# AdrianoEttari/DiffusionRemoteSensing

Hardware: AMD Instinct MI355X
Metric: unet_denoise_steps_per_s (higher is better)
Workload: dtype f16 main + block-scaled fp6 (e2m3) cross terms of tap pairs on the wide 3x3 layers (FL, 11 of 11 launches of the dominant kernel); split bf16 x3 (hi + lo) everywhere else; f32 accumulate

## Files before the change

diffusionremotesensing_amd/csrc/drs_common.h:

```cpp
#pragma once
#include <hip/hip_runtime.h>
#include <stdint.h>
#include <stddef.h>

#include "../../include/drs_hip.h"

#define DRS_MAX_TAPS 9
#define DRS_TAPMODE_CONVT 2

struct TapConv {
  const float* in;
  int in_cs, in_co;
  int N, H, W, Cin;
  const float* w;
  const void* w_aux;
  const float* bias;
  float* out;
  int out_cs, out_co;
  int OH, OW, Cout;
  int TH, TW;
  int in_stride, out_scale, out_oy, out_ox;
  int ntaps;
  int dy[DRS_MAX_TAPS], dx[DRS_MAX_TAPS], wtap[DRS_MAX_TAPS];
  int wtaps_total;
// ... 135 lines not shown
  const float* in; int in_cs, in_co;
  int N, LH, LW, Cc, Ch;
  const void* w;
  const float* bias;
  const float* res; int res_cs, res_co;
  const float* eh;
  const float* ev;
  float* out; int out_cs, out_co;
  float* out2; int out2_cs, out2_co;
  const float* post2; int post2_cs;
  const float* fuse_w; const float* fuse_b; float* fuse_out; int fuse_dim;
  int fuse_acc;
  int proj;
  const void* zero_line;
  unsigned* fault;
};
bool drs_upfuse_proj_supported(int Cc, int Ch, int fuse_dim);
size_t drs_upfuse_proj_weight_bytes(int Cc);
int drs_launch_upfuse_proj_pack(const float* vp, const float* t_w, int Cc, int Ch, int fuse_dim, void* dst, hipStream_t s);
int drs_launch_upfuse_proj(const UpFuseDesc& d, hipStream_t s);
int drs_launch_upfuse_fold_proj(const float* v_w, const float* v_b, const float* fw, const float* fb, int fuse_dim, int Cc, int Ch,
                                float* dst_w, float* dst_b, hipStream_t s);

struct ResBlock0Desc {
  const float* x;
  const void* w1; const float* b1;
  const float* temb; int temb_cs;
  const void* w2; const float* b2;
  const void* ws; const float* bs;
  float* out;
  int N, H, W;
  const void* zero_line;
  unsigned* fault;
};
bool drs_resblock0_supported(int Cin, int Cout, int H, int W);
int drs_launch_resblock0(const ResBlock0Desc& d, hipStream_t s);
struct UpFuseEdgeDesc {
  const float* in; int in_cs, in_co; int N, LH, LW, Cc, Ch;
  const float* rt; const float* rl; const float* bt;
  float* eh; float* ev;
  const void* wimg;
  const void* zero_line;
};
bool drs_upfuse_supported(int Cc, int Ch, int LH, int LW);
size_t drs_upfuse_weight_bytes(int Cc, int Ch);
size_t drs_upfuse_aux_floats(int Cc, int Ch);
size_t drs_upfuse_edge_image_bytes(int Cc, int Ch);
int drs_launch_upfuse_pack(const float* v_w, const float* v_b, const float* t_w, const float* t_b, int Cc, int Ch, void* dst_w,
                           float* dst_aux, void* dst_edge, hipStream_t s);
int drs_launch_upfuse_edges(const UpFuseEdgeDesc& d, hipStream_t s);
int drs_launch_upfuse(const UpFuseDesc& d, hipStream_t s);
int drs_launch_nchw_to_sp(const float* src, float* dst, int N, int C, int H, int W, hipStream_t s);

int drs_launch_sp_add_rowvec(const float* src, float* dst, const float* vec, int vec_stride, int N, long long pix_per_image,
                             int C, hipStream_t s);
bool drs_tapconv_sp8_supported(const TapConv& d, int impl);
bool drs_tapconv_sp_supported(const TapConv& d, int impl);
int drs_launch_conv3x3_direct_sp(const TapConv& d, hipStream_t s);
int drs_launch_fold_proj(const float* w, int cin_total, int cin_off, int Cmid, int Cin, const float* fw, int fuse_dim, float* dst,
// ... 64 lines not shown
```

diffusionremotesensing_amd/csrc/plan.hip:

```cpp
#include <stdarg.h>
#include <stdio.h>
#include <stdlib.h>
#include <string.h>
#include <cxxabi.h>
#include <algorithm>
#include <map>
#include <memory>
#include <mutex>
#include <string>
#include <utility>
#include <vector>

#include "drs_common.h"

static thread_local char g_err[512] = "";
void DrsErr::set(const char* fmt, ...) {
  va_list ap;
  va_start(ap, fmt);
  vsnprintf(g_err, sizeof(g_err), fmt, ap);
  va_end(ap);
}
extern "C" const char* drs_last_error(void) { return g_err; }
extern "C" int drs_abi_version(void) { return 7; }

// ... 377 lines not shown
  int t_PA = -1;
  size_t o_eh = 0, o_ev = 0;
};

}

struct drs_plan {
  drs_unet_config cfg;
  std::vector<Param> params;
  std::vector<ConvLayer*> convs;
  std::vector<PlanarConv*> planars;
  std::vector<Mlp*> mlps;
  std::vector<WsTensor> tensors;

  PlanarConv rrdb[7];
  PlanarConv stem0, stemc;
  ResBlock enc[4];
  ConvLayer downs[3];
  DecStage dec[3];
  ConvLayer output;

  size_t packed_bytes = 0, ws_bytes = 0;
  size_t o_inv_freq = 0, o_mlp_table = 0, o_out_w = 0, o_out_b = 0, o_label = 0, o_zero = 0, o_fault = 0;
  bool sp = false;
  int t_XT[3] = {-1, -1, -1};
  int label_emb = -1;
  int temb_total = 0;
  std::vector<long long> mlp_table_host;
  std::vector<const void*> param_ptrs;
  size_t o_bn_sums = 0, bn_sums_bytes = 0, o_red = 0, red_bytes = 0;
  bool fl = false;
  bool fl_disabled = false;
  int fl_slots = 0;
  size_t o_fl_flags = 0;
  bool packed_ok = false;
  const void* packed_ptr = nullptr;
  unsigned* fault_ptr = nullptr;

  struct OpRec { std::string name; double flops, bytes; hipEvent_t e0, e1; };
  bool profiling = false;
  std::vector<OpRec> ops;
  struct LaunchRec { std::string op, kernel; };
  std::vector<LaunchRec> launches;
  std::string cur_op;

  size_t o_lr[3], o_up, o_temb;
// ... 207 lines not shown
    }
  }
  if (p->fl) {
    for (ConvLayer* L : p->convs)
      if (L->fl_slot >= 0) { L->fl_img_off = cur; cur += align_up(drs_fl_image_bytes(L->Cout, L->Cin, L->taps)); }
    for (int i = 0; i < 2; ++i)
      if (p->dec[i].ah_fl_slot >= 0) { p->dec[i].ah_fl_img_off = cur; cur += align_up(drs_fl_image_bytes(kUp[i + 1], kUp[i + 1], 9)); }
    p->o_fl_flags = cur; cur += align_up((size_t)p->fl_slots * 8);
  }
  for (PlanarConv* L : p->planars) {
    L->w_off = cur; cur += align_up((size_t)L->Cout * L->Cin * 9 * 4);
    L->b_off = cur; cur += align_up((size_t)L->Cout * 4);
  }
  for (Mlp* m : p->mlps) {
    m->o_w1 = cur; cur += align_up((size_t)m->dim * 100 * 4);
    m->o_b1 = cur; cur += align_up((size_t)m->dim * 4);
    m->o_w2 = cur; cur += align_up((size_t)m->dim * m->dim * 4);
    m->o_b2 = cur; cur += align_up((size_t)m->dim * 4);
  }
  p->o_mlp_table = cur; cur += align_up(p->mlps.size() * 6 * sizeof(long long));
  p->o_label = cur; cur += align_up((size_t)(cfg.num_classes > 0 ? cfg.num_classes : 0) * 100 * 4);
  p->o_out_w = cur; cur += align_up((size_t)cfg.out_dim * kUp[3] * 4);
  p->o_out_b = cur; cur += align_up((size_t)cfg.out_dim * 4);
  p->o_zero = cur; cur += 256;
  p->o_fault = cur; cur += 256;
  p->packed_bytes = cur;
}

static void plan_eval_workspace(drs_plan* p, size_t& ws) {
  const drs_unet_config& cfg = p->cfg;
  const int B = cfg.batch, Bl = cfg.lr_batch, H = cfg.height, W = cfg.width, h = H / cfg.magnification, w = W / cfg.magnification;
  const int CCw = cfg.cond_channels > 0 ? cfg.cond_channels : 1;
  for (int i = 0; i < 3; ++i) { p->o_lr[i] = ws; ws += align_up((size_t)Bl * CCw * h * w * 4); }
  p->o_temb = ws; ws += align_up((size_t)B * p->temb_total * 4);
  p->t_lrenc = p->T(cond_encoder_name(cfg), ws, Bl, CCw, h, w, true);
  p->t_up = p->T("upsampled_lr_img", ws, Bl, CCw, H, W, true);
  p->t_cond = p->T("cond", ws, Bl, kDown[0], H, W);
  p->t_x0 = p->T("x0", ws, B, kDown[0], H, W);
  for (int i = 0; i < 4; ++i) {
    const int co = kDown[i + 1], hh = H >> i, ww = W >> i;
    const std::string nm = i < 3 ? "conv_blocks." + std::to_string(i) : std::string("bottle_neck");
    p->t_S[i] = p->T(nm + ".shortcut", ws, B, co, hh, ww);
    if (i == 0) p->t_K0 = p->T(nm + ".skip", ws, B, co, hh, ww);
    p->t_H[i] = p->T(nm + ".h", ws, B, co, hh, ww);
    p->t_R[i] = p->T(nm, ws, B, co, hh, ww);
    if (i < 3) p->t_D[i] = p->T("downs." + std::to_string(i), ws, B, co, hh / 2, ww / 2);
// ... 261 lines not shown
  DRS_CHECK_HIP(hipMemcpyAsync(host.data(), flags, (size_t)plan->fl_slots * 8, hipMemcpyDeviceToHost, c.s));
  DRS_CHECK_HIP(hipStreamSynchronize(c.s));
  for (ConvLayer* L : plan->convs) L->fl_ok = L->fl_slot >= 0 && L->mfma && host[2 * L->fl_slot] == 0u;
  for (DecStage& d : plan->dec) d.ah_fl_ok = d.ah_fl_slot >= 0 && host[2 * d.ah_fl_slot] == 0u;
  return DRS_OK;
}

extern "C" int drs_unet_pack_weights(drs_plan* plan, const void* const* params, const float* inv_freq_host,
                                     void* packed, size_t packed_bytes, drs_stream_t stream) {
  hipStream_t s = (hipStream_t)stream;
  DRS_REQUIRE(plan && params && inv_freq_host && packed, DRS_ERR_ARG, "pack_weights: null pointer");
  DRS_REQUIRE(packed_bytes >= drs_unet_packed_bytes(plan), DRS_ERR_WORKSPACE, "pack_weights: packed buffer too small");
  for (size_t i = 0; i < plan->params.size(); ++i)
    DRS_REQUIRE(params[i], DRS_ERR_ARG, "pack_weights: param %s is null", plan->params[i].name.c_str());
  const PackCtx c{plan, params, aligned_base(packed), s};
  DRS_CHECK_HIP(hipMemcpyAsync(c.base + plan->o_inv_freq, inv_freq_host, 50 * 4, hipMemcpyHostToDevice, s));
  DrsPackQueueScope pack_queue;
  RUN(pack_layers(c));
  RUN(pack_dual_pairs(c));
  RUN(pack_fused_gates(c));
  for (int i = 0; i < 3; ++i)
    if (plan->dec[i].upfuse) RUN(pack_upfuse_stage(c, i));
  RUN(pack_verbatim(c));
  RUN(pack_queue.flush(s));
  if (plan->fl) RUN(pack_fl_images(c));
  DRS_CHECK_HIP(hipMemsetAsync(c.base + plan->o_zero, 0, 512, s));
  plan->param_ptrs.assign(params, params + plan->params.size());
  plan->packed_ok = true;
  plan->packed_ptr = packed;
  return DRS_OK;
}

static void prof_begin(drs_plan* plan, const std::string& name, double flops, double bytes, hipStream_t s) {
  if (!plan->profiling) return;
  drs_plan::OpRec r{name, flops, bytes, nullptr, nullptr};
  (void)hipEventCreate(&r.e0);
  (void)hipEventCreate(&r.e1);
  (void)hipEventRecord(r.e0, s);
  plan->ops.push_back(r);
  plan->cur_op = name;
}
static void prof_end(drs_plan* plan, hipStream_t s) {
  if (!plan->profiling) return;
  (void)hipEventRecord(plan->ops.back().e1, s);
  plan->cur_op.clear();
}
// ... 27 lines not shown
  prof_begin(plan, name, conv_flops(d), conv_bytes(d), s);
  int rc = run_conv(d, L.mfma ? plan->cfg.impl : DRS_IMPL_DIRECT, s);
  if (!rc && split_out2)
    rc = drs_launch_sp_add_rowvec(d_in.out, d_in.out2, d_in.post2, d_in.post2_cs, d_in.N, (long long)d_in.OH * d_in.OW,
                                  d_in.Cout, s);
  prof_end(plan, s);
  return rc;
}

namespace {
struct FwdCtx {
  drs_plan* plan;
  const drs_unet_config& cfg;
  hipStream_t s;
  char* pk;
  void* ws;
  float* temb;
  const void* zero_line;
  float* out;
  int B, H, W, sp;
  bool train;
  bool concurrent = false, mlp_side = false;
  bool xt_only[3] = {false, false, false};
  FwdCtx(drs_plan* p, const void* packed, void* workspace, float* o, hipStream_t stream)
      : plan(p), cfg(p->cfg), s(stream), pk(aligned_base(packed)), ws(aligned_base(workspace)),
        temb((float*)((char*)ws + p->o_temb)), zero_line(pk + p->o_zero), out(o), B(cfg.batch), H(cfg.height),
        W(cfg.width), sp(p->sp ? 1 : 0), train((cfg.flags & DRS_PLAN_TRAIN) != 0) {}
  const float* PW(const ConvLayer& L) const { return (const float*)(pk + L.w_off); }
  const float* PB(const ConvLayer& L) const { return (const float*)(pk + L.b_off); }
  float* TP(int i) const { return plan->tp(ws, i); }
  bool keep_all() const { return (cfg.flags & DRS_PLAN_KEEP_ALL) != 0; }
};
}

template <class Launch>
static int prof_op(drs_plan* plan, const std::string& name, double flops, double bytes, hipStream_t s, Launch launch) {
  prof_begin(plan, name, flops, bytes, s);
  const int rc = launch();
  prof_end(plan, s);
  return rc;
}
static int conv_bn(FwdCtx& f, const ConvLayer& L, const TapConv& d) {
  if (!f.train) return plan_conv(f.plan, L, d, f.s);
  TapConv zc = d;
  zc.out = f.TP(L.t_Z); zc.out_cs = L.Cout; zc.out_co = 0;
  zc.relu_pre = zc.relu_post = 0; zc.post_add = nullptr; zc.res = nullptr;
// ... 66 lines not shown
  }
  const PlanarConv& co = plan->rrdb[6];
  RUN(drs_launch_conv3x3_planar(cur, (const float*)(pk + co.w_off), (const float*)(pk + co.b_off), lr_img,
                                f.TP(plan->t_lrenc), Bl, CC, CC, h, w, 0, s));
  const float* upsrc = f.TP(plan->t_lrenc);
  if (mag > 1 || f.train) {
    RUN(drs_launch_bicubic(f.TP(plan->t_lrenc), f.TP(plan->t_up), Bl, CC, h, w, mag, s));
    upsrc = f.TP(plan->t_up);
  }
  RUN(drs_launch_stem(upsrc, (const float*)(pk + plan->stemc.w_off), (const float*)(pk + plan->stemc.b_off),
                      nullptr, 0, f.TP(plan->t_cond), Bl, CC, kDown[0], H, W, s));
  prof_end(plan, s);
  return DRS_OK;
}
static int fwd_conv0(FwdCtx& f, const float* x, bool has_cond) {
  drs_plan* plan = f.plan;
  const int B = f.B, C = f.cfg.image_channels, H = f.H, W = f.W;
  return prof_op(plan, "conv0", 2.0 * B * H * W * C * kDown[0] * 9, 4.0 * B * H * W * (C + 2.0 * kDown[0]), f.s, [&] {
    return drs_launch_stem(x, (const float*)(f.pk + plan->stem0.w_off), (const float*)(f.pk + plan->stem0.b_off),
                           has_cond ? f.TP(plan->t_cond) : nullptr, f.cfg.lr_batch, f.TP(plan->t_x0), B, C, kDown[0], H, W,
                           f.s, f.sp);
  });
}
static int fwd_encoder_block(FwdCtx& f, int i) {
  drs_plan* plan = f.plan;
  const ResBlock& rb = plan->enc[i];
  const int B = f.B, ci = kDown[i], co = kDown[i + 1], hh = f.H >> i, ww = f.W >> i;
  const float* xin = f.TP(i == 0 ? plan->t_x0 : plan->t_D[i - 1]);
  const bool fuse_shortcut = !f.train && rb.conv2.mfma && rb.shortcut.mfma;
  if (!fuse_shortcut) {
    TapConv d = conv_desc(xin, B, hh, ww, ci, ci, 0, f.PW(rb.shortcut), f.PB(rb.shortcut), f.TP(plan->t_S[i]), co, co, 0,
                          1, 1, 1, 0);
    d.in_sp = f.sp; d.out_sp = rb.shortcut.out_sp ? 1 : 0;
    RUN(conv_bn(f, rb.shortcut, d));
  }
  if (i == 0 && rb.dual && fuse_shortcut && f.sp && !f.keep_all() && f.cfg.impl == DRS_IMPL_MFMA_BF16X3 &&
      drs_resblock0_supported(ci, co, hh, ww)) {
    ResBlock0Desc r0 = {};
    r0.x = xin;
    r0.w1 = f.pk + rb.dual_w_off; r0.b1 = (const float*)(f.pk + rb.dual_b_off);
    r0.temb = f.temb + rb.mlp.temb_off; r0.temb_cs = plan->temb_total;
    r0.w2 = f.PW(rb.conv2); r0.b2 = f.PB(rb.conv2);
    r0.ws = f.PW(rb.shortcut); r0.bs = f.PB(rb.shortcut);
    r0.out = f.TP(plan->t_R[0]);
    r0.N = B; r0.H = hh; r0.W = ww;
    r0.zero_line = f.zero_line; r0.fault = plan->fault_ptr;
    const double px0 = (double)B * hh * ww;
    RUN(prof_op(plan, "conv_blocks.0.fused", 2.0 * px0 * (2.0 * 9 * ci * co + 9.0 * co * co + (double)ci * co),
                4.0 * px0 * (ci + co) + 4.0 * (2.0 * 9 * ci * co + 9.0 * co * co + (double)ci * co), f.s,
                [&] { return drs_launch_resblock0(r0, f.s); }));
  } else {
    bool dual = false;
    if (rb.dual && !f.train && !f.keep_all()) {
      TapConv d = conv_desc(xin, B, hh, ww, ci, ci, 0, (const float*)(f.pk + rb.dual_w_off),
                            (const float*)(f.pk + rb.dual_b_off), f.TP(plan->t_H[i]), co, co, 0, 3, 3, 1, 1);
      d.dual = 1;
      d.relu_pre = 1;
      d.in_sp = d.out_sp = f.sp; d.zero_line = f.zero_line; d.fault = plan->fault_ptr;
      d.post_add = f.temb + rb.mlp.temb_off; d.post_cs = plan->temb_total;
      if (drs_tapconv_ws_supported(d, f.cfg.impl) || drs_tapconv_sp_supported(d, f.cfg.impl)) {
        const std::string& wn = plan->params[rb.conv1.w].name;
        RUN(prof_op(plan, wn.substr(0, wn.size() - 7) + "+skip", 2.0 * conv_flops(d), conv_bytes(d), f.s,
                    [&] { return drs_launch_tapconv_mfma(d, f.cfg.impl, f.s); }));
        dual = true;
      }
    }
    if (rb.has_skip && !dual) {
      TapConv d = conv_desc(xin, B, hh, ww, ci, ci, 0, f.PW(rb.skip), f.PB(rb.skip), f.TP(plan->t_K0), co, co, 0, 3, 3, 1,
                            1);
      d.in_sp = f.sp; d.zero_line = f.zero_line;
      RUN(plan_conv(plan, rb.skip, d, f.s));
    }
// ... 247 lines not shown
  DRS_REQUIRE(!labels || (plan->label_emb >= 0 && (label_batch == plan->cfg.batch || label_batch == 1)), DRS_ERR_ARG,
              "forward: labels need the generation variant with num_classes > 0 and label_batch == batch or 1");
  FwdCtx f(plan, packed, workspace, out, s);
  plan->fault_ptr = (unsigned*)(f.pk + plan->o_fault);
  if (plan->profiling) {
    for (auto& r : plan->ops) { (void)hipEventDestroy(r.e0); (void)hipEventDestroy(r.e1); }
    plan->ops.clear();
  }
  LaunchLogScope launch_log(plan);

  static const int concurrent_env = getenv("DRS_CONCURRENT") ? atoi(getenv("DRS_CONCURRENT")) : -1;
  const bool serial = f.train || plan->profiling || f.cfg.impl == DRS_IMPL_DIRECT;
  f.concurrent = (concurrent_env < 0 ? !plan->sp : concurrent_env != 0) && !serial;
  f.mlp_side = concurrent_env != 0 && !serial;
  if ((f.concurrent || f.mlp_side) && !plan->side) {
    DRS_CHECK_HIP(hipStreamCreateWithFlags(&plan->side, hipStreamNonBlocking));
    for (hipEvent_t* e : {&plan->ev_fork, &plan->ev_join, &plan->ev_gbias, &plan->ev_edge_in[0], &plan->ev_edge_out[0],
                          &plan->ev_edge_in[1], &plan->ev_edge_out[1], &plan->ev_edge_in[2], &plan->ev_edge_out[2]})
      DRS_CHECK_HIP(hipEventCreateWithFlags(e, hipEventDisableTiming));
  }

  RUN(fwd_time_embeddings(f, t, labels, label_batch));
  if (has_cond && !reuse_cond) RUN(fwd_lr_branch(f, lr_img));
  RUN(fwd_conv0(f, x, has_cond));
  if (f.mlp_side) DRS_CHECK_HIP(hipStreamWaitEvent(s, plan->ev_join, 0));
  for (int i = 0; i < 4; ++i) RUN(fwd_encoder_block(f, i));
  if (f.mlp_side) DRS_CHECK_HIP(hipStreamWaitEvent(s, plan->ev_gbias, 0));

  for (int i = 0; i < 3; ++i) {
    const DecStage& st = plan->dec[i];
    if (f.concurrent) {
      DRS_CHECK_HIP(hipEventRecord(plan->ev_fork, s));
      DRS_CHECK_HIP(hipStreamWaitEvent(plan->side, plan->ev_fork, 0));
    }
    const bool edges_aside = st.upfuse && f.mlp_side && !f.concurrent;
    if (edges_aside) {
      RUN(fwd_ups_conv(f, i));
      DRS_CHECK_HIP(hipEventRecord(plan->ev_edge_in[i], s));
      DRS_CHECK_HIP(hipStreamWaitEvent(plan->side, plan->ev_edge_in[i], 0));
      RUN(fwd_attention(f, i));
    } else {
      RUN(fwd_attention(f, i));
      RUN(fwd_ups_conv(f, i));
    }
    RUN(st.upfuse ? fwd_composite_tail(f, i, edges_aside) : fwd_unfused_tail(f, i));
  }
  if (!output_fused(plan)) {
// ... 82 lines not shown
```

diffusionremotesensing_amd/csrc/resblock0_sp.hip:

```cpp
#include <stdio.h>
#include <stdlib.h>

#include "conv_epilogue.h"
#include "mfma_policy.h"
#include "sp_sync.h"

namespace {

constexpr int TW_ = 16, TH_ = 8, IW = TW_ + 2, IH = TH_ + 2, NPIX = IW * IH, NBLK_A = (NPIX + 15) / 16;
constexpr int IMG1 = 5 * 4 * 64 * 16, IMG2 = 36 * 32 * 16, IMGS = 4 * 32 * 16, WIN = NPIX * 128;
constexpr int NPOST = 16;
constexpr int XPLANE = (TH_ + 4) * (TW_ + 4) * 16 + 64, XT = 4 * XPLANE;

#ifdef DRS_SP_TIMELINE
__device__ unsigned long long drs_rb0_tl[32];
#define RB_STAMP(i) do { const unsigned long long t_ = __builtin_amdgcn_s_memtime(); tl[i] += t_ - tl_last; tl_last = t_; } while (0)
#else
#define RB_STAMP(i) do { } while (0)
#endif

__global__ __launch_bounds__(512, 1) void resblock0_kernel(ResBlock0Desc d, unsigned w1_gimage, unsigned w2_gimage,
                                                           unsigned ws_gimage, int debug) {
  extern __shared__ __attribute__((aligned(16))) char smem[];
  using P = PolicyBF16X3;
  using Frag = typename P::Frag;
  auto mfma = [](const bf16x8& w, const bf16x8& x, const f32x4& c) __attribute__((always_inline)) {
    return __builtin_amdgcn_mfma_f32_16x16x32_bf16(w, x, c, 0, 0, 0);
  };
  const int tid = threadIdx.x, lane = tid & 63, wave = __builtin_amdgcn_readfirstlane(tid >> 6);
  const int lr = lane & 15, kg = lane >> 4;
  char* sW1 = smem;
  char* sW2 = sW1 + 2 * IMG1;
  char* sWs = sW2 + 2 * IMG2;
  char* sWinAll = sWs + 2 * IMGS;
  char* sXAll = sWinAll + 2 * WIN;
  float* sB1 = reinterpret_cast<float*>(sXAll + 2 * XT);
  float* sB2 = sB1 + 64;
  unsigned* sCntRaw = reinterpret_cast<unsigned*>(sB2 + 32);
  float* sPost = sB2 + 32 + 8;
  const int npost = min(d.N, NPOST);
  {
    const char* w1 = reinterpret_cast<const char*>(d.w1);
    for (int i = tid; i < 2 * 20 * 64; i += 512) {
      const int im = i >= 20 * 64, idx = im ? i - 20 * 64 : i;
      const int ch = idx % 64, kgp = (idx / 64) & 3, j = idx / (4 * 64), tap = 2 * j + (kgp >> 1);
      u32x4 v = {0u, 0u, 0u, 0u};
// ... 32 lines not shown
  const int qstep_ = 2 * (int)(gridDim.x >> 3);
  const int step_x = qstep_ % gx, step_y = (qstep_ / gx) % gy, step_n = qstep_ / (gx * gy);
  int bx = 0, by = 0;
  auto place_first = [&](int q) __attribute__((always_inline)) {
    bx = q % gx; by = (q / gx) % gy; n = q / (gx * gy);
    tx0 = bx * TW_; ty0 = by * TH_;
  };
  auto place_next = [&]() __attribute__((always_inline)) {
    bx += step_x;
    if (bx >= gx) { bx -= gx; ++by; }
    by += step_y;
    if (by >= gy) { by -= gy; ++n; }
    n += step_n;
    tx0 = bx * TW_; ty0 = by * TH_;
  };
  unsigned goff[4];
#pragma unroll
  for (int i = 0; i < 4; ++i) {
    const int e = i * 256 + gw * 64 + lane, pix = min(e >> 2, XPIX - 1);
    const int py = (pix * 3277) >> 16, px = pix - py * XW;
    goff[i] = (unsigned)((py * d.W + px) * 64 + (e & 3) * 16);
  }
  u32x4 xr[4];
  auto tile_load = [&]() __attribute__((always_inline)) {
    const char* ximg = xb + (size_t)n * d.H * d.W * 64;
    if (ty0 >= 2 && ty0 + TH_ + 2 <= d.H && tx0 >= 2 && tx0 + TW_ + 2 <= d.W) {
      typedef const __attribute__((address_space(1))) char* gptr;
      const unsigned long long gi = (unsigned long long)(ximg + ((long long)(ty0 - 2) * d.W + (tx0 - 2)) * 64);
      gptr g = (gptr)(((unsigned long long)(unsigned)__builtin_amdgcn_readfirstlane((int)(gi >> 32)) << 32) |
                      (unsigned)__builtin_amdgcn_readfirstlane((int)(unsigned)gi));
      asm volatile("" : "+s"(g));
#pragma unroll
      for (int i = 0; i < 4; ++i) xr[i] = *(const __attribute__((address_space(1))) u32x4*)(g + goff[i]);
    } else {
#pragma unroll
      for (int i = 0; i < 4; ++i) {
        const int e = i * 256 + gw * 64 + lane, pix = e >> 2;
        const int py = (pix * 3277) >> 16, px = pix - py * XW;
        const int y = ty0 - 2 + py, x = tx0 - 2 + px;
        const bool ok = pix < XPIX && y >= 0 && y < d.H && x >= 0 && x < d.W;
        xr[i] = *reinterpret_cast<const u32x4*>(ok ? ximg + ((size_t)y * d.W + x) * 64 + (e & 3) * 16 : zero);
      }
    }
  };
  auto tile_store = [&]() __attribute__((always_inline)) {
#pragma unroll
    for (int i = 0; i < 4; ++i) {
      const int e = i * 256 + gw * 64 + lane;
      if ((e >> 2) < XPIX) *reinterpret_cast<u32x4*>(sX + (e & 3) * XPLANE + (e >> 2) * 16) = xr[i];
    }
    sp_release(cTile, lane);
  };
  constexpr int MAXB = NBLK_A / 4;
  static_assert(MAXB * 4 == NBLK_A, "three blocks per wave");
  int wp[MAXB], relL[MAXB], tapL[5];
#pragma unroll
  for (int b = 0; b < MAXB; ++b) {
    const int p = min((gw + 4 * b) * 16 + lr, NPIX - 1);
    const int py = (p * 3641) >> 16, px = p - py * IW;
    wp[b] = p;
    relL[b] = ((py + 1) * XW + px + 1) * 16 + (kg & 1) * XPLANE;
  }
#pragma unroll
  for (int j = 0; j < 5; ++j) {
    const int tap = min(2 * j + (kg >> 1), 8);
    tapL[j] = ((tap / 3 - 1) * XW + tap % 3 - 1) * 16;
  }
  auto operand = [&](int b, int j) __attribute__((always_inline)) {
    const char* p = sX + relL[b] + tapL[j];
    return Frag{*reinterpret_cast<const bf16x8*>(p), *reinterpret_cast<const bf16x8*>(p + 2 * XPLANE)};
  };
  const int q0 = t_lo + 2 * member + grp, qstep = 2 * members;
#ifdef DRS_SP_TIMELINE
  unsigned long long tl[8] = {0, 0, 0, 0, 0, 0, 0, 0};
  const unsigned long long tl_begin = __builtin_amdgcn_s_memtime();
  unsigned long long tl_last = tl_begin, tl_n = 0;
  if ((debug & 1) && grp == 1) return;
#endif
  if (q0 < t_hi) {
    place_first(q0);
    tile_load();
    tile_store();
    if (q0 + qstep < t_hi) {
      place_next();
      tile_load();
      asm volatile("" :: "v"(xr[0]), "v"(xr[1]), "v"(xr[2]), "v"(xr[3]));
    }
  }
  if (grp == 1) { __builtin_amdgcn_s_sleep(64); __builtin_amdgcn_s_sleep(32); }
  unsigned k = 0;
  u32x4 kept[4] = {};
  int cbx = q0 % gx, cby = (q0 / gx) % gy, cn = q0 / (gx * gy);
  for (int q = q0; q < t_hi; q += qstep, ++k) {
#ifdef DRS_SP_TIMELINE
    ++tl_n;
#endif
    RB_STAMP(7);
    const int cty0 = cby * TH_, ctx0 = cbx * TW_;
    sp_poll_lds(cTile, 4u * (k + 1), d.fault);
    const bool more = q + qstep < t_hi;
    f32x4 acc[MAXB][4];
#pragma unroll
    for (int b = 0; b < MAXB; ++b)
#pragma unroll
// ... 38 lines not shown
    }
    asm volatile("" :: "v"(kept[0]), "v"(kept[1]), "v"(kept[2]), "v"(kept[3]));
    RB_STAMP(0);
    Frag xs[2];
#pragma unroll
    for (int r = 0; r < 2; ++r) {
      const char* p = sX + ((2 + 2 * gw + r) * XW + 2 + lr) * 16 + (kg & 1) * XPLANE;
      xs[r] = Frag{*reinterpret_cast<const bf16x8*>(p), *reinterpret_cast<const bf16x8*>(p + 2 * XPLANE)};
    }
    float bm[8], bs[8], te[8];
    {
      const float4 m0 = *reinterpret_cast<const float4*>(sB1 + kg * 8), m1 = *reinterpret_cast<const float4*>(sB1 + kg * 8 + 4);
      const float4 s0 = *reinterpret_cast<const float4*>(sB1 + 32 + kg * 8), s1 = *reinterpret_cast<const float4*>(sB1 + 32 + kg * 8 + 4);
      float4 e0, e1;
      if (cn < npost) {
        e0 = *reinterpret_cast<const float4*>(sPost + cn * 32 + kg * 8); e1 = *reinterpret_cast<const float4*>(sPost + cn * 32 + kg * 8 + 4);
      } else {
        const float* gp = d.temb + (size_t)cn * d.temb_cs + kg * 8;
        e0 = *reinterpret_cast<const float4*>(gp); e1 = *reinterpret_cast<const float4*>(gp + 4);
      }
      bm[0] = m0.x; bm[1] = m0.y; bm[2] = m0.z; bm[3] = m0.w; bm[4] = m1.x; bm[5] = m1.y; bm[6] = m1.z; bm[7] = m1.w;
      bs[0] = s0.x; bs[1] = s0.y; bs[2] = s0.z; bs[3] = s0.w; bs[4] = s1.x; bs[5] = s1.y; bs[6] = s1.z; bs[7] = s1.w;
      te[0] = e0.x; te[1] = e0.y; te[2] = e0.z; te[3] = e0.w; te[4] = e1.x; te[5] = e1.y; te[6] = e1.z; te[7] = e1.w;
    }
    RB_STAMP(1);
    sp_poll_lds(cRead, 4u * k, d.fault);
    RB_STAMP(2);
#pragma unroll
    for (int b = 0; b < MAXB; ++b) {
      float v[8];
#pragma unroll
      for (int t = 0; t < 2; ++t)
#pragma unroll
        for (int i = 0; i < 4; ++i)
          v[t * 4 + i] = (drs_maxf(acc[b][t][i] + bm[t * 4 + i], 0.f) + (acc[b][t + 2][i] + bs[t * 4 + i])) + te[t * 4 + i];
      u32x4 hh, hl;
      drs_sp_split8(v, hh, hl);
      int p = wp[b];
      asm volatile("" : "+v"(p));
      const int py = (p * 3641) >> 16, px = p - py * IW;
      const int y = cty0 - 1 + py, x = ctx0 - 1 + px;
      const bool inside = y >= 0 && y < d.H && x >= 0 && x < d.W;
      if (!inside) { hh = u32x4{0u, 0u, 0u, 0u}; hl = u32x4{0u, 0u, 0u, 0u}; }
      if ((gw + 4 * b) * 16 + lr < NPIX) {
        char* wpix = sWin + p * 128;
        const int s0 = ((kg + p) & 7) * 16;
        *reinterpret_cast<u32x4*>(wpix + s0) = hh;
        *reinterpret_cast<u32x4*>(wpix + (s0 ^ 64)) = hl;
      }
    }
    sp_release(cWritten, lane);
    sp_poll_lds(cWritten, 4u * (k + 1), d.fault);
    if (more) tile_store();
    RB_STAMP(3);
    f32x4 o[2][2];
#pragma unroll
    for (int r = 0; r < 2; ++r)
#pragma unroll
      for (int t = 0; t < 2; ++t) o[r][t] = f32x4{0.f, 0.f, 0.f, 0.f};
    const char* w2lane = sW2 + ((size_t)kg * 32 + lr) * 16;
    auto win = [&](int row, int kx) __attribute__((always_inline)) {
      const int p = (2 * gw + row) * IW + lr + kx;
      const char* wpix = sWin + p * 128;
      const int s0 = ((kg + p) & 7) * 16;
      return Frag{*reinterpret_cast<const bf16x8*>(wpix + s0), *reinterpret_cast<const bf16x8*>(wpix + (s0 ^ 64))};
    };
    Frag wr_[4][3];
    auto win_row = [&](int row) __attribute__((always_inline)) {
#pragma unroll
      for (int kx = 0; kx < 3; ++kx) wr_[row][kx] = win(row, kx);
    };
    win_row(0);
    win_row(1);
    {
// ... 52 lines not shown
        kept[2 * r + 1] = lo ? got : L;
        char* gr = g + (size_t)r * d.W * 128;
        drs_store16(gr, kept[2 * r]);
        drs_store16(gr + 8 * 128, kept[2 * r + 1]);
      }
    }
    RB_STAMP(5);
    cbx += step_x;
    if (cbx >= gx) { cbx -= gx; ++cby; }
    cby += step_y;
    if (cby >= gy) { cby -= gy; ++cn; }
    cn += step_n;
  }
#ifdef DRS_SP_TIMELINE
  if (blockIdx.x == 0 && (wave == 0 || wave == 7) && lane == 0) {
    const int o = wave == 0 ? 0 : 16;
    for (int i = 0; i < 8; ++i) drs_rb0_tl[o + i] = tl[i];
    drs_rb0_tl[o + 8] = tl_n;
    drs_rb0_tl[o + 9] = __builtin_amdgcn_s_memtime() - tl_begin;
  }
#endif
}

size_t resblock0_lds(int N) { return (size_t)2 * (IMG1 + IMG2 + IMGS) + 2 * WIN + 2 * XT + (size_t)(64 + 32 + 8 + 32 * (N < NPOST ? N : NPOST)) * 4; }

}

bool drs_resblock0_supported(int Cin, int Cout, int H, int W) {
  static const bool env = !(getenv("DRS_RB0") && atoi(getenv("DRS_RB0")) == 0);
  return env && Cin == 16 && Cout == 32 && H >= 32 && W >= 32 && H % TH_ == 0 && W % TW_ == 0;
}

int drs_launch_resblock0(const ResBlock0Desc& d, hipStream_t s) {
  DRS_REQUIRE(drs_resblock0_supported(16, 32, d.H, d.W), DRS_ERR_SHAPE, "resblock0: H=%d W=%d", d.H, d.W);
  DRS_REQUIRE(d.x && d.w1 && d.b1 && d.temb && d.w2 && d.b2 && d.ws && d.bs && d.out && d.zero_line, DRS_ERR_ARG, "resblock0: null pointer");
  if (d.N == 0) return DRS_OK;
  int num_cu = 0;
  {
    const int rc = drs_kernel_prepare(reinterpret_cast<const void*>(resblock0_kernel), 160 * 1024, &num_cu);
    if (rc) return rc;
  }
  const unsigned w1_gimage = 9u * 4u * 64u * 16u, w2_gimage = 9u * 4u * 32u * 16u, ws_gimage = 4u * 32u * 16u;
  const int blocks = num_cu / 8 * 8;
  DRS_LAUNCH(resblock0_kernel, dim3((unsigned)blocks), dim3(512), resblock0_lds(d.N), s, d, w1_gimage, w2_gimage, ws_gimage, 0);
  DRS_CHECK_HIP(hipGetLastError());
#ifdef DRS_SP_TIMELINE
  {
    unsigned long long h[32];
    const int dbg = getenv("DRS_RB0_DEBUG") ? atoi(getenv("DRS_RB0_DEBUG")) : 0;
    hipEvent_t e0, e1;
    float ms = 0.f;
    DRS_CHECK_HIP(hipEventCreate(&e0)); DRS_CHECK_HIP(hipEventCreate(&e1));
    DRS_CHECK_HIP(hipEventRecord(e0, s));
    DRS_LAUNCH(resblock0_kernel, dim3((unsigned)blocks), dim3(512), resblock0_lds(d.N), s, d, w1_gimage, w2_gimage, ws_gimage, dbg);
    DRS_CHECK_HIP(hipEventRecord(e1, s));
    DRS_CHECK_HIP(hipStreamSynchronize(s));
    DRS_CHECK_HIP(hipEventElapsedTime(&ms, e0, e1));
    (void)hipEventDestroy(e0); (void)hipEventDestroy(e1);
    DRS_CHECK_HIP(hipMemcpyFromSymbol(h, HIP_SYMBOL(drs_rb0_tl), sizeof(h)));
    for (int w = 0; w < 2; ++w) {
      const unsigned long long* t = h + 16 * w;
      const double sc = t[8] ? 1.0 / (double)t[8] : 0.0;
      fprintf(stderr, "resblock0 %dx%d wave %d: %.1f us, %llu patches, alive %llu ticks (%.0f / patch) | top %.0f  A-mfma %.0f  A-epi %.0f  bar1 %.0f  "
              "winstore+bar2 %.0f  B-mfma %.0f  B-epi %.0f\n", d.H, d.W, w ? 7 : 0, ms * 1e3, t[8], t[9], t[9] * sc, t[7] * sc, t[0] * sc, t[1] * sc,
              t[2] * sc, t[3] * sc, t[4] * sc, t[5] * sc);
    }
  }
#endif
  return DRS_OK;
}
```

Before: 819.7.

## Fuse stem 3x3 conv into the persistent resblock0 kernel

```diff
diff --git a/diffusionremotesensing_amd/csrc/drs_common.h b/diffusionremotesensing_amd/csrc/drs_common.h
--- a/diffusionremotesensing_amd/csrc/drs_common.h
+++ b/diffusionremotesensing_amd/csrc/drs_common.h
@@ -181,8 +181,12 @@
 int drs_launch_upfuse_fold_proj(const float* v_w, const float* v_b, const float* fw, const float* fb, int fuse_dim, int Cc, int Ch,
                                 float* dst_w, float* dst_b, hipStream_t s);
 
+constexpr int kResBlock0StemBands = 4;
 struct ResBlock0Desc {
   const float* x;
+  const float* img; int img_channels;
+  const float* stem_tab;
+  const float* cond; int cond_batch;
   const void* w1; const float* b1;
   const float* temb; int temb_cs;
   const void* w2; const float* b2;
@@ -194,6 +198,8 @@
 };
 bool drs_resblock0_supported(int Cin, int Cout, int H, int W);
 int drs_launch_resblock0(const ResBlock0Desc& d, hipStream_t s);
+bool drs_resblock0_stem_supported(int image_channels);
+int drs_launch_resblock0_stem_table(const float* w, const float* b, float* dst, int C, hipStream_t s);
 struct UpFuseEdgeDesc {
   const float* in; int in_cs, in_co; int N, LH, LW, Cc, Ch;
   const float* rt; const float* rl; const float* bt;
diff --git a/diffusionremotesensing_amd/csrc/plan.hip b/diffusionremotesensing_amd/csrc/plan.hip
--- a/diffusionremotesensing_amd/csrc/plan.hip
+++ b/diffusionremotesensing_amd/csrc/plan.hip
@@ -423,6 +423,7 @@
 
   size_t packed_bytes = 0, ws_bytes = 0;
   size_t o_inv_freq = 0, o_mlp_table = 0, o_out_w = 0, o_out_b = 0, o_label = 0, o_zero = 0, o_fault = 0;
+  size_t o_rb0_stem = 0;
   bool sp = false;
   int t_XT[3] = {-1, -1, -1};
   int label_emb = -1;
@@ -676,6 +677,9 @@
   p->o_label = cur; cur += align_up((size_t)(cfg.num_classes > 0 ? cfg.num_classes : 0) * 100 * 4);
   p->o_out_w = cur; cur += align_up((size_t)cfg.out_dim * kUp[3] * 4);
   p->o_out_b = cur; cur += align_up((size_t)cfg.out_dim * 4);
+  if (p->sp && cfg.image_channels <= kResBlock0StemBands) {
+    p->o_rb0_stem = cur; cur += align_up((size_t)(cfg.image_channels * 144 + 16) * 4);
+  }
   p->o_zero = cur; cur += 256;
   p->o_fault = cur; cur += 256;
   p->packed_bytes = cur;
@@ -983,6 +987,9 @@
   for (int i = 0; i < 3; ++i)
     if (plan->dec[i].upfuse) RUN(pack_upfuse_stage(c, i));
   RUN(pack_verbatim(c));
+  if (plan->o_rb0_stem)
+    RUN(drs_launch_resblock0_stem_table(c.F(plan->stem0.w), c.F(plan->stem0.b), (float*)(c.base + plan->o_rb0_stem),
+                                        plan->cfg.image_channels, s));
   RUN(pack_queue.flush(s));
   if (plan->fl) RUN(pack_fl_images(c));
   DRS_CHECK_HIP(hipMemsetAsync(c.base + plan->o_zero, 0, 512, s));
@@ -1056,6 +1063,9 @@
   bool train;
   bool concurrent = false, mlp_side = false;
   bool xt_only[3] = {false, false, false};
+  const float* x_img = nullptr;
+  bool has_cond = false;
+  bool stem_fused = false;
   FwdCtx(drs_plan* p, const void* packed, void* workspace, float* o, hipStream_t stream)
       : plan(p), cfg(p->cfg), s(stream), pk(aligned_base(packed)), ws(aligned_base(workspace)),
         temb((float*)((char*)ws + p->o_temb)), zero_line(pk + p->o_zero), out(o), B(cfg.batch), H(cfg.height),
@@ -1168,6 +1178,11 @@
                            f.s, f.sp);
   });
 }
+static bool block0_one_launch(const FwdCtx& f) {
+  const ResBlock& rb = f.plan->enc[0];
+  return rb.dual && !f.train && rb.conv2.mfma && rb.shortcut.mfma && f.sp && !f.keep_all() &&
+         f.cfg.impl == DRS_IMPL_MFMA_BF16X3 && drs_resblock0_supported(kDown[0], kDown[1], f.H, f.W);
+}
 static int fwd_encoder_block(FwdCtx& f, int i) {
   drs_plan* plan = f.plan;
   const ResBlock& rb = plan->enc[i];
@@ -1180,10 +1195,19 @@
     d.in_sp = f.sp; d.out_sp = rb.shortcut.out_sp ? 1 : 0;
     RUN(conv_bn(f, rb.shortcut, d));
   }
-  if (i == 0 && rb.dual && fuse_shortcut && f.sp && !f.keep_all() && f.cfg.impl == DRS_IMPL_MFMA_BF16X3 &&
-      drs_resblock0_supported(ci, co, hh, ww)) {
+  if (i == 0 && block0_one_launch(f)) {
     ResBlock0Desc r0 = {};
     r0.x = xin;
+    double stem_flops = 0.0, stem_bytes = 0.0;
+    if (f.stem_fused) {
+      const int C = f.cfg.image_channels;
+      r0.x = nullptr;
+      r0.img = f.x_img; r0.img_channels = C;
+      r0.stem_tab = (const float*)(f.pk + plan->o_rb0_stem);
+      r0.cond = f.has_cond ? f.TP(plan->t_cond) : nullptr; r0.cond_batch = f.cfg.lr_batch;
+      stem_flops = 2.0 * B * hh * ww * C * kDown[0] * 9;
+      stem_bytes = 4.0 * B * hh * ww * C + (f.has_cond ? 4.0 * f.cfg.lr_batch * hh * ww * kDown[0] : 0.0) - 4.0 * B * hh * ww * ci;
+    }
     r0.w1 = f.pk + rb.dual_w_off; r0.b1 = (const float*)(f.pk + rb.dual_b_off);
     r0.temb = f.temb + rb.mlp.temb_off; r0.temb_cs = plan->temb_total;
     r0.w2 = f.PW(rb.conv2); r0.b2 = f.PB(rb.conv2);
@@ -1192,8 +1216,8 @@
     r0.N = B; r0.H = hh; r0.W = ww;
     r0.zero_line = f.zero_line; r0.fault = plan->fault_ptr;
     const double px0 = (double)B * hh * ww;
-    RUN(prof_op(plan, "conv_blocks.0.fused", 2.0 * px0 * (2.0 * 9 * ci * co + 9.0 * co * co + (double)ci * co),
-                4.0 * px0 * (ci + co) + 4.0 * (2.0 * 9 * ci * co + 9.0 * co * co + (double)ci * co), f.s,
+    RUN(prof_op(plan, "conv_blocks.0.fused", stem_flops + 2.0 * px0 * (2.0 * 9 * ci * co + 9.0 * co * co + (double)ci * co),
+                stem_bytes + 4.0 * px0 * (ci + co) + 4.0 * (2.0 * 9 * ci * co + 9.0 * co * co + (double)ci * co), f.s,
                 [&] { return drs_launch_resblock0(r0, f.s); }));
   } else {
     bool dual = false;
@@ -1487,7 +1511,9 @@
 
   RUN(fwd_time_embeddings(f, t, labels, label_batch));
   if (has_cond && !reuse_cond) RUN(fwd_lr_branch(f, lr_img));
-  RUN(fwd_conv0(f, x, has_cond));
+  f.x_img = x; f.has_cond = has_cond;
+  f.stem_fused = plan->o_rb0_stem != 0 && block0_one_launch(f) && drs_resblock0_stem_supported(f.cfg.image_channels);
+  if (!f.stem_fused) RUN(fwd_conv0(f, x, has_cond));
   if (f.mlp_side) DRS_CHECK_HIP(hipStreamWaitEvent(s, plan->ev_join, 0));
   for (int i = 0; i < 4; ++i) RUN(fwd_encoder_block(f, i));
   if (f.mlp_side) DRS_CHECK_HIP(hipStreamWaitEvent(s, plan->ev_gbias, 0));
diff --git a/diffusionremotesensing_amd/csrc/resblock0_sp.hip b/diffusionremotesensing_amd/csrc/resblock0_sp.hip
--- a/diffusionremotesensing_amd/csrc/resblock0_sp.hip
+++ b/diffusionremotesensing_amd/csrc/resblock0_sp.hip
@@ -19,9 +19,15 @@
 #define RB_STAMP(i) do { } while (0)
 #endif
 
-__global__ __launch_bounds__(512, 1) void resblock0_kernel(ResBlock0Desc d, unsigned w1_gimage, unsigned w2_gimage,
-                                                           unsigned ws_gimage, int debug) {
+typedef float F3 __attribute__((ext_vector_type(3), aligned(4)));
+
+template <int C>
+__device__ __forceinline__ void resblock0_body(const ResBlock0Desc& d, unsigned w1_gimage, unsigned w2_gimage,
+                                               unsigned ws_gimage, int debug) {
   extern __shared__ __attribute__((aligned(16))) char smem[];
+  constexpr bool STEM = C > 0;
+  constexpr int CS = STEM ? C : 1;
+  constexpr bool XEARLY = C <= 3;
   using P = PolicyBF16X3;
   using Frag = typename P::Frag;
   auto mfma = [](const bf16x8& w, const bf16x8& x, const f32x4& c) __attribute__((always_inline)) {
@@ -100,7 +106,80 @@
     goff[i] = (unsigned)((py * d.W + px) * 64 + (e & 3) * 16);
   }
   u32x4 xr[4];
+  const int sL = gw * 64 + lane, sU = min(sL >> 2, XPIX / 4 - 1), sBand = (sU * 3277) >> 16;
+  const int spy = sBand * 4 + (sL & 3), spx = sU - sBand * XW;
+  const bool sHas = (sL >> 2) < XPIX / 4;
+  static_assert(XPIX / 4 * 4 == XPIX && (TH_ + 4) % 4 == 0, "units of four rows");
+  typedef const __attribute__((address_space(4))) float* cfptr;
+  const cfptr stab = (cfptr)(unsigned long long)d.stem_tab;
+  F3 xin[CS][3];
+  auto x_load = [&]() __attribute__((always_inline)) {
+    const int y0 = ty0 - 3 + spy, x = tx0 - 3 + spx;
+    const float* img = d.img + (size_t)n * C * d.H * d.W;
+    if (ty0 >= 3 && ty0 + TH_ + 3 <= d.H && tx0 >= 3 && tx0 + TW_ + 3 <= d.W) {
+      const float* ip = img + (long long)y0 * d.W + x;
+#pragma unroll
+      for (int ci = 0; ci < CS; ++ci)
+#pragma unroll
+        for (int r = 0; r < 3; ++r)
+          xin[ci][r] = *reinterpret_cast<const F3*>(ip + ((size_t)ci * d.H + r) * d.W);
+    } else {
+#pragma unroll
+      for (int ci = 0; ci < CS; ++ci)
+#pragma unroll
+        for (int r = 0; r < 3; ++r) {
+          const int y = y0 + r;
+          const bool yok = y >= 0 && y < d.H;
+#pragma unroll
+          for (int kx = 0; kx < 3; ++kx)
+            xin[ci][r][kx] = *((yok && x + kx >= 0 && x + kx < d.W) ? img + ((size_t)ci * d.H + y) * d.W + x + kx : reinterpret_cast<const float*>(zero));
+        }
+    }
+  };
+  auto conv0_tile = [&]() __attribute__((always_inline)) {
+    drs_f32x2 acc[8];
+#pragma unroll
+    for (int j = 0; j < 8; ++j) acc[j] = *reinterpret_cast<const __attribute__((address_space(4))) drs_f32x2*>(stab + C * 144 + 2 * j);
+#pragma unroll
+    for (int ci = 0; ci < CS; ++ci)
+#pragma unroll
+      for (int t = 0; t < 9; ++t) {
+        const float a = xin[ci][t / 3][t % 3];
+        const drs_f32x2 a2 = {a, a};
+#pragma unroll
+        for (int j = 0; j < 8; ++j)
+          acc[j] = __builtin_elementwise_fma(a2, *reinterpret_cast<const __attribute__((address_space(4))) drs_f32x2*>(stab + (ci * 9 + t) * 16 + 2 * j), acc[j]);
+      }
+    if (d.cond) {
+#pragma unroll
+      for (int i = 0; i < 4; ++i) {
+        acc[2 * i] += drs_f32x2{__uint_as_float(xr[i][0]), __uint_as_float(xr[i][1])};
+        acc[2 * i + 1] += drs_f32x2{__uint_as_float(xr[i][2]), __uint_as_float(xr[i][3])};
+      }
+    }
+    const int y = ty0 - 2 + spy, x = tx0 - 2 + spx;
+    const bool inside = y >= 0 && y < d.H && x >= 0 && x < d.W;
+#pragma unroll
+    for (int h = 0; h < 2; ++h)
+#pragma unroll
+      for (int q = 0; q < 4; ++q) {
+        const uint2 s_ = drs_split2(acc[4 * h + q][0], acc[4 * h + q][1]);
+        xr[h][q] = inside ? s_.x : 0u;
+        xr[2 + h][q] = inside ? s_.y : 0u;
+      }
+  };
   auto tile_load = [&]() __attribute__((always_inline)) {
+    if (STEM) {
+      if (!d.cond) return;
+      const char* cimg = reinterpret_cast<const char*>(d.cond) + (d.cond_batch == 1 ? (size_t)0 : (size_t)n * d.H * d.W * 64);
+      const int y = ty0 - 2 + spy, x = tx0 - 2 + spx;
+      const bool inner = ty0 >= 2 && ty0 + TH_ + 2 <= d.H && tx0 >= 2 && tx0 + TW_ + 2 <= d.W;
+      const bool ok = inner || (sHas && y >= 0 && y < d.H && x >= 0 && x < d.W);
+      const char* p = ok ? cimg + ((long long)y * d.W + x) * 64 : zero;
+#pragma unroll
+      for (int i = 0; i < 4; ++i) xr[i] = *reinterpret_cast<const u32x4*>(p + i * 16);
+      return;
+    }
     const char* ximg = xb + (size_t)n * d.H * d.W * 64;
     if (ty0 >= 2 && ty0 + TH_ + 2 <= d.H && tx0 >= 2 && tx0 + TW_ + 2 <= d.W) {
       typedef const __attribute__((address_space(1))) char* gptr;
@@ -122,6 +201,14 @@
     }
   };
   auto tile_store = [&]() __attribute__((always_inline)) {
+    if (STEM) {
+      if (sHas) {
+#pragma unroll
+        for (int i = 0; i < 4; ++i) *reinterpret_cast<u32x4*>(sX + i * XPLANE + (spy * XW + spx) * 16) = xr[i];
+      }
+      sp_release(cTile, lane);
+      return;
+    }
 #pragma unroll
     for (int i = 0; i < 4; ++i) {
       const int e = i * 256 + gw * 64 + lane;
@@ -158,6 +245,7 @@
   if (q0 < t_hi) {
     place_first(q0);
     tile_load();
+    if (STEM) { x_load(); conv0_tile(); }
     tile_store();
     if (q0 + qstep < t_hi) {
       place_next();
@@ -242,6 +330,10 @@
       bm[0] = m0.x; bm[1] = m0.y; bm[2] = m0.z; bm[3] = m0.w; bm[4] = m1.x; bm[5] = m1.y; bm[6] = m1.z; bm[7] = m1.w;
       bs[0] = s0.x; bs[1] = s0.y; bs[2] = s0.z; bs[3] = s0.w; bs[4] = s1.x; bs[5] = s1.y; bs[6] = s1.z; bs[7] = s1.w;
       te[0] = e0.x; te[1] = e0.y; te[2] = e0.z; te[3] = e0.w; te[4] = e1.x; te[5] = e1.y; te[6] = e1.z; te[7] = e1.w;
+    }
+    if (STEM && XEARLY) {
+      asm volatile("" :: "v"(te[0]), "v"(te[1]), "v"(te[2]), "v"(te[3]), "v"(te[4]), "v"(te[5]), "v"(te[6]), "v"(te[7]));
+      if (more) x_load();
     }
     RB_STAMP(1);
     sp_poll_lds(cRead, 4u * k, d.fault);
@@ -270,6 +362,8 @@
       }
     }
     sp_release(cWritten, lane);
+    if (STEM && !XEARLY && more) x_load();
+    if (STEM && more) conv0_tile();
     sp_poll_lds(cWritten, 4u * (k + 1), d.fault);
     if (more) tile_store();
     RB_STAMP(3);
@@ -368,6 +462,22 @@
 #endif
 }
 
+__global__ __launch_bounds__(512, 1) void resblock0_kernel(ResBlock0Desc d, unsigned w1_gimage, unsigned w2_gimage,
+                                                           unsigned ws_gimage, int debug) {
+  resblock0_body<0>(d, w1_gimage, w2_gimage, ws_gimage, debug);
+}
+template <int C>
+__global__ __launch_bounds__(512, 1) void resblock0_stem_kernel(ResBlock0Desc d, unsigned w1_gimage, unsigned w2_gimage,
+                                                                unsigned ws_gimage, int debug) {
+  resblock0_body<C>(d, w1_gimage, w2_gimage, ws_gimage, debug);
+}
+
+__global__ void resblock0_stem_table_kernel(const float* __restrict__ w, const float* __restrict__ b, float* __restrict__ dst, int C) {
+  const int i = blockIdx.x * blockDim.x + threadIdx.x;
+  if (i < C * 144) dst[i] = w[((i & 15) * C + i / 144) * 9 + (i / 16) % 9];
+  else if (i < C * 144 + 16) dst[i] = b[i - C * 144];
+}
+
 size_t resblock0_lds(int N) { return (size_t)2 * (IMG1 + IMG2 + IMGS) + 2 * WIN + 2 * XT + (size_t)(64 + 32 + 8 + 32 * (N < NPOST ? N : NPOST)) * 4; }
 
 }
@@ -377,18 +487,40 @@
   return env && Cin == 16 && Cout == 32 && H >= 32 && W >= 32 && H % TH_ == 0 && W % TW_ == 0;
 }
 
+bool drs_resblock0_stem_supported(int image_channels) {
+  static const bool env = !(getenv("DRS_RB0_STEM") && atoi(getenv("DRS_RB0_STEM")) == 0);
+  return env && image_channels >= 1 && image_channels <= kResBlock0StemBands;
+}
+
+int drs_launch_resblock0_stem_table(const float* w, const float* b, float* dst, int C, hipStream_t s) {
+  DRS_REQUIRE(w && b && dst && C >= 1 && C <= kResBlock0StemBands, DRS_ERR_ARG, "resblock0 stem table: C=%d", C);
+  DRS_LAUNCH(resblock0_stem_table_kernel, dim3((unsigned)drs_cdiv(C * 144 + 16, 256)), dim3(256), 0, s, w, b, dst, C);
+  DRS_CHECK_HIP(hipGetLastError());
+  return DRS_OK;
+}
+
 int drs_launch_resblock0(const ResBlock0Desc& d, hipStream_t s) {
   DRS_REQUIRE(drs_resblock0_supported(16, 32, d.H, d.W), DRS_ERR_SHAPE, "resblock0: H=%d W=%d", d.H, d.W);
-  DRS_REQUIRE(d.x && d.w1 && d.b1 && d.temb && d.w2 && d.b2 && d.ws && d.bs && d.out && d.zero_line, DRS_ERR_ARG, "resblock0: null pointer");
+  typedef void (*Kern)(ResBlock0Desc, unsigned, unsigned, unsigned, int);
+  Kern kern = resblock0_kernel;
+  if (d.img) {
+    DRS_REQUIRE(d.stem_tab && d.img_channels >= 1 && d.img_channels <= kResBlock0StemBands && (!d.cond || d.cond_batch == 1 || d.cond_batch == d.N),
+                DRS_ERR_ARG, "resblock0 stem: bands=%d cond_batch=%d N=%d", d.img_channels, d.cond_batch, d.N);
+    static const Kern stem[kResBlock0StemBands] = {resblock0_stem_kernel<1>, resblock0_stem_kernel<2>, resblock0_stem_kernel<3>, resblock0_stem_kernel<4>};
+    kern = stem[d.img_channels - 1];
+  } else {
+    DRS_REQUIRE(d.x, DRS_ERR_ARG, "resblock0: null pointer");
+  }
+  DRS_REQUIRE(d.w1 && d.b1 && d.temb && d.w2 && d.b2 && d.ws && d.bs && d.out && d.zero_line, DRS_ERR_ARG, "resblock0: null pointer");
   if (d.N == 0) return DRS_OK;
   int num_cu = 0;
   {
-    const int rc = drs_kernel_prepare(reinterpret_cast<const void*>(resblock0_kernel), 160 * 1024, &num_cu);
+    const int rc = drs_kernel_prepare(reinterpret_cast<const void*>(kern), 160 * 1024, &num_cu);
     if (rc) return rc;
   }
   const unsigned w1_gimage = 9u * 4u * 64u * 16u, w2_gimage = 9u * 4u * 32u * 16u, ws_gimage = 4u * 32u * 16u;
   const int blocks = num_cu / 8 * 8;
-  DRS_LAUNCH(resblock0_kernel, dim3((unsigned)blocks), dim3(512), resblock0_lds(d.N), s, d, w1_gimage, w2_gimage, ws_gimage, 0);
+  DRS_LAUNCH(kern, dim3((unsigned)blocks), dim3(512), resblock0_lds(d.N), s, d, w1_gimage, w2_gimage, ws_gimage, 0);
   DRS_CHECK_HIP(hipGetLastError());
 #ifdef DRS_SP_TIMELINE
   {
@@ -398,7 +530,7 @@
     float ms = 0.f;
     DRS_CHECK_HIP(hipEventCreate(&e0)); DRS_CHECK_HIP(hipEventCreate(&e1));
     DRS_CHECK_HIP(hipEventRecord(e0, s));
-    DRS_LAUNCH(resblock0_kernel, dim3((unsigned)blocks), dim3(512), resblock0_lds(d.N), s, d, w1_gimage, w2_gimage, ws_gimage, dbg);
+    DRS_LAUNCH(kern, dim3((unsigned)blocks), dim3(512), resblock0_lds(d.N), s, d, w1_gimage, w2_gimage, ws_gimage, dbg);
     DRS_CHECK_HIP(hipEventRecord(e1, s));
     DRS_CHECK_HIP(hipStreamSynchronize(s));
     DRS_CHECK_HIP(hipEventElapsedTime(&ms, e0, e1));
```

New measurement: 818.1. Within noise of the previous version (-0.2%).
